# lukecavabarrett/pna

Measured on NVIDIA H100. Metric: aggregated edges/sec (PNA layer fwd), higher is better.
Workload: dtype f32

## Files before the change

### include/pna_b200.h

```cpp
#ifndef PNA_B200_H
#define PNA_B200_H

#include <stddef.h>
#include <stdint.h>

#ifdef __cplusplus
extern "C" {
#endif

#define PNA_ABI_VERSION 8

typedef void* pna_stream_t;

enum pna_status {
  PNA_OK = 0,
  PNA_ERR_BAD_ARG = -1,
  PNA_ERR_UNSUPPORTED = -2,
  PNA_ERR_CUDA = -3,
  PNA_ERR_INDEX = -4,
  PNA_ERR_WORKSPACE = -5,
  PNA_ERR_CAPTURING = -6
};

enum pna_dtype { PNA_F32 = 0, PNA_BF16 = 1 };

enum pna_aggr { PNA_AGGR_SUM = 0, PNA_AGGR_MEAN = 1, PNA_AGGR_MIN = 2, PNA_AGGR_MAX = 3, PNA_AGGR_VAR = 4, PNA_AGGR_STD = 5,
                PNA_AGGR_MOMENT3 = 6, PNA_AGGR_MOMENT4 = 7, PNA_AGGR_MOMENT5 = 8,
                PNA_AGGR_SOFTMAX = 9, PNA_AGGR_SOFTMIN = 10, PNA_AGGR_NORMALISED_MEAN = 11,
                PNA_AGGR_SKIP = 15  };
enum pna_scaler { PNA_SCALE_IDENTITY = 0, PNA_SCALE_AMPLIFICATION = 1, PNA_SCALE_ATTENUATION = 2, PNA_SCALE_LINEAR = 3, PNA_SCALE_INVERSE_LINEAR = 4 };

#define PNA_MAX_AGGR 6
#define PNA_MAX_SCALERS 5

enum pna_flags {
  PNA_FLAG_ZERO_ISOLATED = 1u,
  PNA_FLAG_SKIP_LIGHT = 2u,
  PNA_FLAG_SKIP_HUBS = 4u,
  PNA_FLAG_GATHER_L1 = 16u,
  PNA_FLAG_RELU_VAR = 8u
};

enum pna_query_what {
  PNA_QUERY_ABI_VERSION = 0,
  PNA_QUERY_SM_ARCH = 1,
  PNA_QUERY_DEFAULT_SPLIT = 2,
  PNA_QUERY_DEFAULT_CHUNK = 3,
  PNA_QUERY_DEVICE_SM_COUNT = 4,
  PNA_QUERY_MAX_FEATURES = 5,
  PNA_QUERY_SIZEOF_CSR = 6,
  PNA_QUERY_SIZEOF_AGG = 7
};

typedef struct pna_csr {
  int64_t n_nodes;
  int64_t n_edges;
  int32_t split_threshold;
  int32_t chunk_edges;
  int32_t* rowptr;
  int32_t* col;
  int32_t* perm;
  int32_t* hub_info;
  int32_t* chunk_items;
  int64_t cap_hubs;
  int64_t cap_chunks;
  int64_t n_hubs;
  int64_t n_chunks;
  int32_t max_degree;
  int32_t n_part;
  int32_t* light_rowptr;
  int32_t* light_deg;
  int32_t* light_col;
// ... 154 lines not shown
```

### pna_b200/_lib.py

```python
from __future__ import annotations

import ctypes as C
import os
import subprocess
import threading

_HERE = os.path.dirname(os.path.abspath(__file__))
REPO_ROOT = os.path.dirname(_HERE)
LIB_PATH = os.environ.get("PNA_B200_LIB") or os.path.join(_HERE, "libpna_sm90.so")
CUDA_SOURCES = [os.path.join(_HERE, "csrc", n) for n in
                ("pna_aggregate.cu", "pna_aggregate_f32_vec.cu", "pna_aggregate_f32_scalar.cu", "pna_aggregate_bf16_vec.cu",
                 "pna_aggregate_bf16_scalar.cu", "pna_aggregate_bwd.cu", "pna_linear.cu", "pna_csr.cu", "pna_peer.cu", "pna_misc.cu",
                 "pna_edge_mlp.cu")]
CUDA_HEADERS = [os.path.join(_HERE, "csrc", n) for n in ("common.cuh", "pna_aggregate.cuh", "pna_aggregate_impl.cuh",
                                                                   "pna_aggregate_moments.cuh", "pna_aggregate_weighted.cuh")] + [
    os.path.join(REPO_ROOT, "include", "pna_b200.h")]
BUILD_DIR = os.path.join(_HERE, "csrc", "build")

NVCC_FLAGS = ["-gencode", "arch=compute_90a,code=sm_90a", "-lineinfo", "-O3", "-std=c++17", "-fmad=false", "-Xcompiler", "-fPIC"]

ABI_VERSION = 8
PNA_OK = 0
PNA_ERR_CAPTURING = -6
PNA_F32, PNA_BF16 = 0, 1
AGGR_CODES = {"sum": 0, "mean": 1, "min": 2, "max": 3, "var": 4, "std": 5, "_skip": 15}
MOMENTS = ("moment3", "moment4", "moment5")
WEIGHTED = ("softmax", "softmin", "normalised_mean")
ALL_AGGR_CODES = {**AGGR_CODES, "moment3": 6, "moment4": 7, "moment5": 8, "softmax": 9, "softmin": 10, "normalised_mean": 11}
SCALER_CODES = {"identity": 0, "amplification": 1, "attenuation": 2, "linear": 3, "inverse_linear": 4}
FLAG_ZERO_ISOLATED, FLAG_SKIP_LIGHT, FLAG_SKIP_HUBS, FLAG_RELU_VAR, FLAG_GATHER_L1 = 1, 2, 4, 8, 16
(QUERY_ABI_VERSION, QUERY_SM_ARCH, QUERY_DEFAULT_SPLIT, QUERY_DEFAULT_CHUNK, QUERY_DEVICE_SM_COUNT,
 QUERY_MAX_FEATURES, QUERY_SIZEOF_CSR, QUERY_SIZEOF_AGG) = range(8)
EDGE_MLP_MAX_WIDTH = 64

EXPORTED_SYMBOLS = ("pna_csr_workspace_bytes", "pna_csr_build", "pna_csr_light_view", "pna_csr_light_view_workspace_bytes", "pna_aggregate_fwd", "pna_aggregate_bwd",
                    "pna_aggregate_bwd_coef", "pna_aggregate_bwd_combine", "pna_aggregate_bwd_slots", "pna_aggregate_bwd_peer_slots",
                    "pna_gather_rows", "pna_halo_pull", "pna_halo_grad_pull", "pna_peer_barrier", "pna_linear_fwd", "pna_linear_scaled_fwd", "pna_row_scales", "pna_linear_workspace_bytes",
                    "pna_linear_bwd_workspace_bytes", "pna_linear_bwd_data", "pna_linear_bwd_weight", "pna_edge_mlp_fwd",
                    "pna_edge_mlp_bwd", "pna_edge_msg_fwd", "pna_edge_msg_bwd", "pna_query", "pna_last_error",
                    "pna_linear_towers_scaled_fwd", "pna_linear_towers_bwd_data", "pna_edge_msg_fwd_bf16", "pna_edge_msg_bwd_bf16",
                    "pna_linear_towers_scaled_fwd_bf16")


class PnaError(RuntimeError):

    def __init__(self, status: int, message: str):
        super().__init__(f"libpna_sm90 status {status}: {message}")
        self.status = status


class CsrStruct(C.Structure):
    _fields_ = [
        ("n_nodes", C.c_int64), ("n_edges", C.c_int64),
        ("split_threshold", C.c_int32), ("chunk_edges", C.c_int32),
        ("rowptr", C.c_void_p), ("col", C.c_void_p), ("perm", C.c_void_p),
        ("hub_info", C.c_void_p), ("chunk_items", C.c_void_p),
        ("cap_hubs", C.c_int64), ("cap_chunks", C.c_int64),
        ("n_hubs", C.c_int64), ("n_chunks", C.c_int64),
        ("max_degree", C.c_int32), ("n_part", C.c_int32),
        ("light_rowptr", C.c_void_p), ("light_deg", C.c_void_p), ("light_col", C.c_void_p), ("part", C.c_void_p),
        ("n_light_edges", C.c_int64), ("n_src_nodes", C.c_int64), ("hot_source_fraction", C.c_float), ("reserved", C.c_int32),
    ]

# ... 190 lines not shown
```

### pna_b200/aggregate.py

```python
from __future__ import annotations

import ctypes as C
import os
from typing import Mapping, Optional, Sequence, Union

import torch

from . import _lib, capture
from .csr import CSRGraph

_DTYPES = {torch.float32: _lib.PNA_F32, torch.bfloat16: _lib.PNA_BF16}
Names = Union[str, Sequence[str]]


def _names(v: Names) -> list:
    return v.split() if isinstance(v, str) else list(v)


def _ptr(t: Optional[torch.Tensor]):
    return None if t is None else t.data_ptr()


def _rows2d(t: torch.Tensor, what: str) -> torch.Tensor:
    if t.dim() != 2:
        raise ValueError(f"{what} must be 2-D, got shape {tuple(t.shape)}")
    if t.size(1) > 1 and t.stride(1) != 1:
        t = t.contiguous()
    if t.size(0) > 1 and t.stride(0) < t.size(1):
        t = t.contiguous()
    return t


HOT_SOURCE_FRACTION_FOR_L1 = 0.25


DYNAMIC_TAIL_MIN_PARTITION_COST = 256


def _dynamic_tail(csr: CSRGraph) -> bool:
    return csr.n_part > 0 and (csr.n_edges + 12 * csr.n_nodes) / csr.n_part >= DYNAMIC_TAIL_MIN_PARTITION_COST


def _check_scaler_degree(t: torch.Tensor, n_rows: int, dev) -> torch.Tensor:
    if t.dtype != torch.int32 or t.device != dev or t.numel() != n_rows or not t.is_contiguous():
        raise ValueError("scaler_degree must be a contiguous int32 [n_rows] tensor on the same device")
    return t


def _check_degree_col(t: torch.Tensor, n_edges: int, dev) -> torch.Tensor:
    if t.dtype != torch.int32 or t.device != dev or t.numel() != n_edges or not t.is_contiguous():
        raise ValueError("degree_col must be a contiguous int32 [n_edges] tensor on the same device")
    return t


def fold_finalize_enabled() -> bool:
    return os.environ.get("PNA_B200_FOLD_FINALIZE", "0") == "1"


def boundary_dtype() -> Optional[torch.dtype]:
    if not torch.is_autocast_enabled("cuda"):
        return None
    return torch.bfloat16 if torch.get_autocast_dtype("cuda") == torch.bfloat16 else torch.float32


def at_boundary(t: Optional[torch.Tensor]) -> Optional[torch.Tensor]:
    if t is not None and t.dtype == torch.float16 and boundary_dtype() is not None:
        return t.float()
    return t

# ... 27 lines not shown
    N = csr.n_nodes
    if F % towers != 0:
        raise ValueError(f"feature width {F} not divisible by towers={towers}")
    Ft = F // towers
    if messages_in_csr_order:
        if gathered.size(0) != csr.n_edges:
            raise ValueError("messages_in_csr_order needs one row per CSR slot")
    n_aggr, aggr_codes = _lib.pack_codes(aggregators, _lib.ALL_AGGR_CODES, "aggregator")
    n_scal, scal_codes = _lib.pack_codes(scalers, _lib.SCALER_CODES, "scaler")
    if row_bias is not None:
        row_bias = _rows2d(row_bias.to(gathered.dtype), "row_bias")
        if tuple(row_bias.shape) != (N, F):
            raise ValueError(f"row_bias must be [{N}, {F}]")
    if self_feat is not None:
        self_feat = _rows2d(self_feat.to(gathered.dtype), "self_feat")
        need = F if self_divided else Ft
        if self_feat.size(0) != N or self_feat.size(1) != need:
            raise ValueError(f"self_feat must be [{N}, {need}]")
    width = towers * output_width(Ft, n_aggr, n_scal, self_feat is not None)
    if out is None:
        out = torch.empty((N, width), dtype=gathered.dtype, device=dev)
    else:
        if out.dtype != gathered.dtype or out.device != dev or out.dim() != 2 or out.size(0) != N or out.size(1) < width \
                or out.stride(1) != 1:
            raise ValueError("bad `out` buffer")
    if row_ids is not None:
        if row_ids.dtype != torch.int32 or not row_ids.is_contiguous() or row_ids.device != dev:
            raise ValueError("row_ids must be a contiguous int32 tensor on the same device")
    if gather_l1 is None:
        gather_l1 = (not messages_in_csr_order) and peer is None and csr.hot_source_fraction > HOT_SOURCE_FRACTION_FOR_L1
    flags = (_lib.FLAG_GATHER_L1 if gather_l1 else 0) | \
            (_lib.FLAG_ZERO_ISOLATED if zero_isolated else 0) | (_lib.FLAG_SKIP_LIGHT if skip_light else 0) | \
            (_lib.FLAG_SKIP_HUBS if skip_hubs else 0) | (_lib.FLAG_RELU_VAR if relu_var else 0)
    partials = None if skip_hubs else csr.hub_partials(F)
    d = _lib.AggStruct(
        gathered=_ptr(gathered), ld_gathered=gathered.stride(0) if gathered.size(0) > 1 else F,
        rowptr=_ptr(csr.rowptr), col=None if messages_in_csr_order else (_ptr(csr.col) if csr.n_edges else None),
        row_bias=_ptr(row_bias), ld_row_bias=0 if row_bias is None else (row_bias.stride(0) if N > 1 else F),
        self_feat=_ptr(self_feat), ld_self=0 if self_feat is None else (self_feat.stride(0) if N > 1 else self_feat.size(1)),
        self_tower_stride=Ft if (self_feat is not None and self_divided) else 0,
        out=_ptr(out), ld_out=out.stride(0) if N > 1 else out.size(1),
        n_rows=N, n_feat=F, n_towers=towers, dtype=_DTYPES[gathered.dtype],
        n_aggr=n_aggr, aggr_codes=aggr_codes, n_scalers=n_scal, scaler_codes=scal_codes,
        avg_log=float(avg_deg["log"]), avg_lin=float(avg_deg.get("lin", 1.0)),
        flags=flags, split_threshold=csr.split_threshold, chunk_edges=csr.chunk_edges,
        hub_info=_ptr(csr.hub_info) if csr.n_hubs else None, chunk_items=_ptr(csr.chunk_items) if csr.n_hubs else None,
        n_hubs=csr.n_hubs, n_chunks=csr.n_chunks, hub_partials=_ptr(partials), max_degree=int(csr.max_degree),
        row_ids=_ptr(row_ids), n_row_ids=0 if row_ids is None else int(row_ids.numel()))
    if scaler_degree is not None:
        d.scaler_degree = _check_scaler_degree(scaler_degree, N, dev).data_ptr()
    if degree_col is not None:
        d.degree_col = _check_degree_col(degree_col, csr.n_edges, dev).data_ptr()
    if view is None and row_ids is None and _dynamic_tail(csr):
        d.work_counter = _ptr(csr.work_counter())
    if view is None and row_ids is None:
        view = csr.full_view()
        if fold_finalize_enabled() and not skip_hubs and peer is None:
            d.hub_done = _ptr(csr.hub_done())
    if view is not None and row_ids is None and N > 0:
        d.light_rowptr, d.light_deg, d.part, d.n_part = _ptr(view.light_rowptr), _ptr(view.light_deg), _ptr(view.part), view.n_part
        d.light_col = _ptr(view.light_col) if csr.n_edges else None
        d.n_view_rows = view.n_view_rows or N
    if peer is not None:
        ptr_table, shift = peer
        if ptr_table.dtype != torch.int64 or ptr_table.device != dev:
            raise ValueError("peer pointer table must be an int64 tensor on the same device")
# ... 194 lines not shown
```

### pna_b200/csrc/common.cuh

```cuda
#pragma once
#include <cuda_runtime.h>
#include <cuda_bf16.h>
#include <stdint.h>
#include <stdio.h>
#include <stdarg.h>
#include "../../include/pna_b200.h"

#if defined(__CUDA_ARCH__) && (__CUDA_ARCH__ != 900)
#error "libpna_sm90 is written for sm_90a (H100) only"
#endif

namespace pna {

void set_error(const char* fmt, ...);
int cuda_fail(cudaError_t e, const char* what);

#define PNA_CUDA_TRY(expr)                                   \
  do {                                                       \
    cudaError_t _e = (expr);                                 \
    if (_e != cudaSuccess) return ::pna::cuda_fail(_e, #expr); \
  } while (0)

#define PNA_REQUIRE(cond, code, ...)      \
  do {                                    \
// ... 32 lines not shown
    }
  }
};
__device__ __forceinline__ DegScales deg_scales(int deg, float avg_log, float avg_lin) {
  const bool iso = deg == 0;
  const float degf = (float)deg;
  const float lg = logf(degf + 1.0f);
  DegScales s;
  s.amp = __fdiv_rn(lg, avg_log);
  s.att = iso ? 1.0f : __fdiv_rn(avg_log, lg);
  s.lin = __fdiv_rn(degf, avg_lin);
  s.ilin = iso ? 1.0f : __fdiv_rn(avg_lin, degf);
  return s;
}

template <typename V>
__device__ __forceinline__ void store_out(V* p, V v) { __stcs(p, v); }

template <typename T, int VEC>
struct Io;

template <>
struct Io<float, 4> {
  typedef float4 Raw;
  static __device__ __forceinline__ Raw load_raw(const float* p) { return __ldg(reinterpret_cast<const float4*>(p)); }
  static __device__ __forceinline__ void unpack(const Raw& r, float (&v)[4]) { v[0] = r.x; v[1] = r.y; v[2] = r.z; v[3] = r.w; }
  static __device__ __forceinline__ void load(const float* p, float (&v)[4]) { unpack(load_raw(p), v); }
  static __device__ __forceinline__ void store(float* p, const float (&v)[4]) {
    store_out(reinterpret_cast<float4*>(p), make_float4(v[0], v[1], v[2], v[3]));
  }
};

template <>
struct Io<float, 1> {
  typedef float Raw;
  static __device__ __forceinline__ Raw load_raw(const float* p) { return __ldg(p); }
  static __device__ __forceinline__ void unpack(const Raw& r, float (&v)[1]) { v[0] = r; }
  static __device__ __forceinline__ void load(const float* p, float (&v)[1]) { v[0] = __ldg(p); }
  static __device__ __forceinline__ void store(float* p, const float (&v)[1]) { __stcs(p, v[0]); }
};

template <>
struct Io<__nv_bfloat16, 8> {
  typedef uint4 Raw;
  static __device__ __forceinline__ Raw load_raw(const __nv_bfloat16* p) { return __ldg(reinterpret_cast<const uint4*>(p)); }
  static __device__ __forceinline__ void load(const __nv_bfloat16* p, float (&v)[8]) { unpack(load_raw(p), v); }
  static __device__ __forceinline__ void unpack(const Raw& r, float (&v)[8]) {
    v[0] = __uint_as_float(r.x << 16); v[1] = __uint_as_float(r.x & 0xffff0000u);
    v[2] = __uint_as_float(r.y << 16); v[3] = __uint_as_float(r.y & 0xffff0000u);
    v[4] = __uint_as_float(r.z << 16); v[5] = __uint_as_float(r.z & 0xffff0000u);
    v[6] = __uint_as_float(r.w << 16); v[7] = __uint_as_float(r.w & 0xffff0000u);
  }
  static __device__ __forceinline__ unsigned pack(float lo, float hi) {
    const __nv_bfloat162 b = __floats2bfloat162_rn(lo, hi);
    return *reinterpret_cast<const unsigned*>(&b);
  }
  static __device__ __forceinline__ void store(__nv_bfloat16* p, const float (&v)[8]) {
    uint4 r;
    r.x = pack(v[0], v[1]); r.y = pack(v[2], v[3]); r.z = pack(v[4], v[5]); r.w = pack(v[6], v[7]);
    store_out(reinterpret_cast<uint4*>(p), r);
  }
};

template <>
struct Io<__nv_bfloat16, 1> {
  typedef unsigned short Raw;
// ... 11 lines not shown
```

### pna_b200/csrc/pna_aggregate_impl.cuh

```cuda
#pragma once
#include "pna_aggregate.cuh"

namespace pna {

constexpr int kThreads = 256;
constexpr int min_blocks(int vec, int k) { return vec * k <= 4 ? 4 : (vec * k <= 8 ? 3 : (vec * k <= 16 ? 2 : 1)); }

template <int VEC>
__device__ __forceinline__ void store_f32(float* p, const float (&v)[VEC]) {
  if constexpr (VEC % 4 == 0) {
#pragma unroll
    for (int i = 0; i < VEC; i += 4) *reinterpret_cast<float4*>(p + i) = make_float4(v[i], v[i + 1], v[i + 2], v[i + 3]);
  } else {
#pragma unroll
    for (int i = 0; i < VEC; ++i) p[i] = v[i];
  }
}

template <typename T, int VEC, int G, int K, int U, typename Cfg>
__global__ void __launch_bounds__(kThreads, min_blocks(VEC, K)) k_rows(const KParams p) {
  constexpr int RPW = 32 / G;
  const int lane = threadIdx.x & 31;
  const int gl = lane % G;
  const long long slot = ((long long)blockIdx.x * (kThreads / 32) + (threadIdx.x >> 5)) * RPW + lane / G;
  long long row;
  if (p.row_ids) {
    if (slot >= p.n_row_ids) return;
    row = __ldg(p.row_ids + slot);
  } else {
    if (slot >= p.n_rows) return;
    row = slot;
  }
  const int beg = __ldg(p.rowptr + row), end = __ldg(p.rowptr + row + 1);
// ... 158 lines not shown
              }
            }
        }
      }
    }

#pragma unroll
    for (int u = 0; u < U; ++u) {
      const int src = __shfl_sync(FULL, cvN, gbase + u);
      if (u < dN) {
#pragma unroll
        for (int k = 0; k < K; ++k)
          if (fm.ok[k]) raw[u][k] = Io<T, VEC>::load_raw((PEER ? gathered_row<T>(p, src) : local_row<T>(p, src)) + fm.f[k]);
      }
    }
    if (deg >= 0) finalize_row_ds<T, VEC, G, K, Cfg>(p, fm, (long long)row, deg, scales_of_row(s_scale_lut, p, row, deg), acc);

    row = rowN; beg = begN; deg = degN; d = dN; cv = cvN;
    if (has_bias) {
#pragma unroll
      for (int k = 0; k < K; ++k)
#pragma unroll
        for (int i = 0; i < VEC; ++i) bias[BIAS ? k : 0][i] = biasN[BIAS ? k : 0][i];
    }
  }
}

constexpr int kStreamThreads = 128;

__device__ __forceinline__ unsigned smem_u32(const void* ptr) { return (unsigned)__cvta_generic_to_shared(ptr); }

template <typename T, int VEC>
__device__ __forceinline__ typename Io<T, VEC>::Raw lds_raw(unsigned addr) {
  static_assert(sizeof(typename Io<T, VEC>::Raw) == 16, "the stream path moves 128-bit chunks");
  typename Io<T, VEC>::Raw r;
  unsigned* w = reinterpret_cast<unsigned*>(&r);
  unsigned a, b, c, d;
  asm volatile("ld.shared.v4.b32 {%0, %1, %2, %3}, [%4];" : "=r"(a), "=r"(b), "=r"(c), "=r"(d) : "r"(addr));
  w[0] = a; w[1] = b; w[2] = c; w[3] = d;
  return r;
}

template <typename T, int VEC, int K, int DEPTH = 1>
struct StreamGeom {
  static constexpr int kHalfBytes = 4096;
  static constexpr int kStages = 2;
  static constexpr int kBlockBytes = 32 * VEC * K * (int)sizeof(T);
  static constexpr int kHalf = kHalfBytes * DEPTH;
  static constexpr int kH = (kHalf / kBlockBytes) < 4 ? 4 : ((kHalf / kBlockBytes) > 32 ? 32 : (kHalf / kBlockBytes));
  static constexpr int kWarpBytes = kStages * kH * kBlockBytes;
  static constexpr size_t kSmem = (size_t)(kStreamThreads / 32) * kWarpBytes;
};

template <bool L1 = false>
__device__ __forceinline__ void cp_async16(unsigned dst, const void* src, unsigned long long policy) {
  if constexpr (L1)
    asm volatile("cp.async.ca.shared.global.L2::cache_hint [%0], [%1], 16, %2;" ::"r"(dst), "l"(__cvta_generic_to_global(src)), "l"(policy)
                 : "memory");
  else
    asm volatile("cp.async.cg.shared.global.L2::cache_hint [%0], [%1], 16, %2;" ::"r"(dst), "l"(__cvta_generic_to_global(src)), "l"(policy)
                 : "memory");
}
__device__ __forceinline__ void cp_async_commit() { asm volatile("cp.async.commit_group;" ::: "memory"); }
template <int N>
__device__ __forceinline__ void cp_async_wait() { asm volatile("cp.async.wait_group %0;" ::"n"(N) : "memory"); }
__device__ __forceinline__ unsigned long long l2_policy_evict_last() {
  unsigned long long pol;
  asm volatile("createpolicy.fractional.L2::evict_last.b64 %0, 1.0;" : "=l"(pol));
  return pol;
}

constexpr int kFinGroups = 8;

template <int VEC, int K, int UF>
__device__ __forceinline__ void merge_partials(const float* __restrict__ base, long long F, const int (&f)[K], const bool (&ok)[K],
                                               int first, int count, int stride, Acc<VEC> (&acc)[K]) {
  for (int j = 0; j < count; j += UF) {
    float ps[UF][K][4][VEC];
#pragma unroll
    for (int u = 0; u < UF; ++u) {
// ... 57 lines not shown
    if (lane == 0) t = atomicAdd(ctr, 1);
    return __shfl_sync(FULL, t, 0);
  };
  if (nch > kFinGroups) {
    const int g = jc % kFinGroups;
    const int mine = (nch - g + kFinGroups - 1) / kFinGroups;
    if (arrive(cnt + g) != mine - 1) return;
    if (lane == 0) cnt[g] = 0;
    __threadfence();
#pragma unroll
    for (int k = 0; k < K; ++k) acc[k].init();
    merge_partials<VEC, K, UFm>(p.partials, p.F, fm.f, fm.ok, first + g, mine, kFinGroups, acc);
    float* __restrict__ part = p.partials + (long long)(first + g) * 4ll * p.F;
#pragma unroll
    for (int k = 0; k < K; ++k) {
      if (!fm.ok[k]) continue;
      store_f32<VEC>(part + 0ll * p.F + fm.f[k], acc[k].sum);
      store_f32<VEC>(part + 1ll * p.F + fm.f[k], acc[k].sq);
      store_f32<VEC>(part + 2ll * p.F + fm.f[k], acc[k].mn);
      store_f32<VEC>(part + 3ll * p.F + fm.f[k], acc[k].mx);
    }
    if (arrive(cnt + 8) != kFinGroups - 1) return;
  } else if (arrive(cnt + 8) != nch - 1) {
    return;
  }
  if (lane == 0) cnt[8] = 0;
  __threadfence();
#pragma unroll
  for (int k = 0; k < K; ++k) acc[k].init();
  merge_partials<VEC, K, UFm>(p.partials, p.F, fm.f, fm.ok, first, nch > kFinGroups ? kFinGroups : nch, 1, acc);
  finalize_row<T, VEC, G, K, Cfg>(p, fm, (long long)__ldg(p.hub_info + 4 * h), __ldg(p.hub_info + 4 * h + 3), acc);
}

template <typename T, int VEC, int K, typename Cfg, bool BIAS, int DEPTH, bool FOLD = false, bool L1 = false>
__global__ void __launch_bounds__(kStreamThreads, tiled_min_blocks(VEC, K)) k_rows_stream(const __grid_constant__ KParams p) {
  constexpr int G = 32;
  constexpr int H = StreamGeom<T, VEC, K, DEPTH>::kH;
  constexpr int SLOT = StreamGeom<T, VEC, K, DEPTH>::kBlockBytes;
  constexpr int NST = StreamGeom<T, VEC, K, DEPTH>::kStages;
  constexpr int CB = 16;
  constexpr unsigned FULL = 0xffffffffu;
  constexpr bool PEER = DEPTH > 1;
  extern __shared__ __align__(128) unsigned char smem[];
  __shared__ float4 s_scale_lut[kScaleLut];
  const int lane = threadIdx.x & 31;
  const int warp = threadIdx.x >> 5;
  fill_scale_lut(s_scale_lut, p, threadIdx.x, kStreamThreads);

  const unsigned ring = smem_u32(smem) + warp * StreamGeom<T, VEC, K, DEPTH>::kWarpBytes;
  const unsigned long long keep = l2_policy_evict_last();

  const long long W = (long long)gridDim.x * (kStreamThreads / 32);
  const long long w = (long long)blockIdx.x * (kStreamThreads / 32) + warp;
  const int n_static = p.work_ctr ? p.n_static : p.n_part;
  int pi_a = (int)((w * n_static) / W), pi_b = (int)(((w + 1) * n_static) / W);
#pragma unroll 1
 for (;;) {
  const int pa = __ldg(p.part + pi_a);
  const int pb = __ldg(p.part + pi_b);
  const int Q0 = __ldg(p.lrowptr + pa);
  const int Te = __ldg(p.lrowptr + pb) - Q0;
  if (pa < pb) {
  const int* __restrict__ lcol = p.lcol + Q0;
  const int fblock = blockIdx.y * (G * VEC * K);
  FeatMap<VEC, G, K> fm;
  fm.init(p, lane, fblock);

  auto source_of = [&](int q) -> int { return (lane < H && q < Te) ? __ldg(lcol + q) : 0; };
  const int lane_elems = fblock + lane * VEC;
  const char* const xlane = reinterpret_cast<const char*>(static_cast<const T*>(p.x) + lane_elems);
  const unsigned ldxb = (unsigned)p.ldx * (unsigned)sizeof(T);
  auto issue_half = [&](int stage, int src) {
    unsigned dst = ring + (unsigned)(stage * H) * SLOT + lane * CB;
#pragma unroll
    for (int u = 0; u < H; ++u, dst += SLOT) {
      const int s_u = __shfl_sync(FULL, src, u);
      const char* sp;
      if constexpr (PEER) sp = reinterpret_cast<const char*>(gathered_row<T>(p, s_u) + lane_elems);
      else sp = xlane + (unsigned long long)(unsigned)s_u * ldxb;
#pragma unroll
      for (int k = 0; k < K; ++k)
        if (fm.ok[k]) cp_async16<L1>(dst + k * (32 * CB), sp + k * (32 * CB), keep);
    }
    cp_async_commit();
  };

  int pend = source_of(lane);
  if (Te > 0) {
#pragma unroll
    for (int s0 = 0; s0 < NST; ++s0) {
      issue_half(s0, pend);
      pend = source_of((s0 + 1) * H + lane);
    }
  }
  int stage = 0;
  int n_issued = NST;

  auto load_deg = [&](int r) -> int { return (r + lane < pb) ? __ldg(p.ldeg + r + lane) : -1; };
  const ViewMap vmap = {p.n_rows, (int)(p.n_view_rows - p.n_rows)};
  auto load_rid = [&](int r) -> int {
    if (p.row_ids) return (r + lane < pb) ? __ldg(p.row_ids + r + lane) : 0;
    return (int)vmap.to_row(r + lane);
  };
  int dg = load_deg(pa), rid = load_rid(pa);

  const unsigned lane_off = (unsigned)lane * (unsigned)CB;
  int q = 0;
#pragma unroll 1
  for (int r0 = pa; r0 < pb; r0 += 32) {
    const int dgN = load_deg(r0 + 32), ridN = load_rid(r0 + 32);
    const int nj = min(32, pb - r0);
#pragma unroll 1
    for (int j = 0; j < nj; ++j) {
      const int deg = __shfl_sync(FULL, dg, j);
      if (deg < 0) continue;
      const int row = __shfl_sync(FULL, rid, j);
      const bool chunk_row = row >= p.n_rows;
      float bias[BIAS ? K : 1][VEC];
      if (BIAS) {
        long long brow = row;
        if (chunk_row) brow = __ldg(p.hub_info + 4 * __ldg(p.chunk_items + 2 * (row - (int)p.n_rows)));
#pragma unroll
        for (int k = 0; k < K; ++k)
          if (fm.ok[k]) Io<T, VEC>::load(static_cast<const T*>(p.bias) + brow * p.ldb + fm.f[k], bias[BIAS ? k : 0]);
      }
      Acc<VEC> acc[K];
#pragma unroll
      for (int k = 0; k < K; ++k) acc[k].init();

      int left = deg;
      while (left > 0) {
        const int inhalf = q & (H - 1);
        if (inhalf == 0) {
          cp_async_wait<NST - 1>();
        }
        const int seg = min(left, H - inhalf);
        unsigned sp = ring + (unsigned)(stage * H + inhalf) * SLOT + lane_off;
        int t = 0;
        for (; t + 2 <= seg; t += 2, sp += 2 * SLOT) {
#pragma unroll
          for (int k = 0; k < K; ++k) {
            if (fm.ok[k]) {
              float m0[VEC], m1[VEC];
              Io<T, VEC>::unpack(lds_raw<T, VEC>(sp + k * (32 * CB)), m0);
              Io<T, VEC>::unpack(lds_raw<T, VEC>(sp + SLOT + k * (32 * CB)), m1);
              acc[k].template add2<BIAS>(m0, m1, bias[BIAS ? k : 0]);
            }
          }
        }
        if (t < seg) {
#pragma unroll
          for (int k = 0; k < K; ++k) {
            if (fm.ok[k]) {
              float m0[VEC];
              Io<T, VEC>::unpack(lds_raw<T, VEC>(sp + k * (32 * CB)), m0);
              acc[k].template add1<BIAS>(m0, bias[BIAS ? k : 0]);
            }
          }
        }
        q += seg;
        left -= seg;
        if ((q & (H - 1)) == 0 || q == Te) {
          issue_half(stage, pend);
          pend = source_of((n_issued + 1) * H + lane);
          ++n_issued;
          stage = (stage + 1 == NST) ? 0 : stage + 1;
        }
      }
      if (!chunk_row) {
        if (Cfg::kStatic && deg == 0 && !p.sdeg) {
          finalize_isolated_row<T, VEC, G, K, Cfg>(p, fm, (long long)row, scales_of_row(s_scale_lut, p, row, 0));
        } else {
          finalize_row_ds<T, VEC, G, K, Cfg>(p, fm, (long long)row, deg, scales_of_row(s_scale_lut, p, row, deg), acc);
        }
      } else {
        float* __restrict__ part = p.partials + (long long)(row - (int)p.n_rows) * 4ll * p.F;
#pragma unroll
        for (int k = 0; k < K; ++k) {
          if (!fm.ok[k]) continue;
          store_f32<VEC>(part + 0ll * p.F + fm.f[k], acc[k].sum);
          store_f32<VEC>(part + 1ll * p.F + fm.f[k], acc[k].sq);
          store_f32<VEC>(part + 2ll * p.F + fm.f[k], acc[k].mn);
          store_f32<VEC>(part + 3ll * p.F + fm.f[k], acc[k].mx);
        }
        if constexpr (FOLD) fold_split_row<T, VEC, K, Cfg>(p, row - (int)p.n_rows, fblock);
      }
    }
    dg = dgN; rid = ridN;
  }
  if (p.work_ctr) { cp_async_wait<0>(); __syncwarp(); }
  }
  if (!p.work_ctr) break;
  int g = 0;
  if (lane == 0) g = atomicAdd(p.work_ctr, 1);
  g = __shfl_sync(FULL, g, 0);
  pi_a = n_static + g;
  if (pi_a >= p.n_part) break;
  pi_b = pi_a + 1;
 }
}

template <typename T, int VEC, int G, int K, int U>
__global__ void __launch_bounds__(kThreads, min_blocks(VEC, K)) k_hub_chunks(const KParams p) {
  constexpr int RPW = 32 / G;
  const int lane = threadIdx.x & 31;
  const int gl = lane % G;
  const long long c = ((long long)blockIdx.x * (kThreads / 32) + (threadIdx.x >> 5)) * RPW + lane / G;
  if (c >= p.n_chunks) return;
  const int h = __ldg(p.chunk_items + 2 * c), j = __ldg(p.chunk_items + 2 * c + 1);
  const long long row = __ldg(p.hub_info + 4 * h);
  const int rbeg = __ldg(p.rowptr + row), rend = __ldg(p.rowptr + row + 1);
  const int beg = rbeg + j * p.chunk;
  const int end = min(beg + p.chunk, rend);

  FeatMap<VEC, G, K> fm;
  fm.init(p, gl, blockIdx.y * (G * VEC * K));
  Acc<VEC> acc[K];
  float bias[K][VEC];
#pragma unroll
  for (int k = 0; k < K; ++k) {
    acc[k].init();
    if (p.bias && fm.ok[k]) Io<T, VEC>::load(static_cast<const T*>(p.bias) + row * p.ldb + fm.f[k], bias[k]);
  }
// ... 141 lines not shown
    if (q != 0) return;
#pragma unroll
    for (int k = 0; k < K; ++k) acc[k].init();
    merge_partials<VEC, K, UF>(p.partials, p.F, fm.f, fm.ok, first, kFinGroups, 1, acc);
  } else {
    if (q != 0) return;
    merge_partials<VEC, K, UF>(p.partials, p.F, fm.f, fm.ok, first, nch, 1, acc);
  }
  finalize_row<T, VEC, G, K, CfgDynamic>(p, fm, row, deg, acc);
}

template <typename T, int VEC, int G, int K, int U>
static int launch_config(const KParams& p_in, cudaStream_t st) {
  constexpr int RPW = 32 / G;
  constexpr int per_block = (kThreads / 32) * RPW;
  KParams p = p_in;
  const unsigned gy = (unsigned)((p.F + G * VEC * K - 1) / (G * VEC * K));
  if (gy != 1 || !(p.n_view_rows > p.n_rows) || p.hub_merged) p.hub_done = nullptr;
  bool folded = false;
  bool chunks_in_stream = false;
  if (!(p.flags & PNA_FLAG_SKIP_LIGHT)) {
    const long long slots = p.row_ids ? p.n_row_ids : p.n_rows;
    if (slots > 0) {
      const long long gx = (slots + per_block - 1) / per_block;
      PNA_REQUIRE(gx <= 0x7fffffffll, PNA_ERR_UNSUPPORTED, "too many rows for one launch: %lld", slots);
      const unsigned std_s = (0u) | (1u << 4) | (2u << 8);
      const bool s3 = p.nS == 3 && (p.scodes & 0xfffu) == std_s && p.nA == 4;
      const bool s1 = p.nS == 1 && (p.scodes & 0xfu) == PNA_SCALE_IDENTITY && p.nA == 4;
      const int cfg = (p.acodes & 0xffffu) != CfgMeanMaxMinStd::ACODES ? 0 : s3 ? 1 : s1 ? 2 : 0;
      if (G == 32 && VEC > 1 && p.lrowptr != nullptr && p.col != nullptr) {
       if constexpr (G == 32 && VEC > 1) {
        const bool b = p.bias != nullptr;
        const bool deep = p.peer_x != nullptr;
#define PNA_LAUNCH_STREAM_(CFG, B, DEPTH, FOLD) PNA_LAUNCH_STREAM__(CFG, B, DEPTH, FOLD, false)
#define PNA_LAUNCH_STREAM__(CFG, B, DEPTH, FOLD, L1)                                                                    \
  do {                                                                                                             \
    constexpr size_t smem = StreamGeom<T, VEC, K, DEPTH>::kSmem;                                                   \
    auto kern = k_rows_stream<T, VEC, K, CFG, B, DEPTH, FOLD, L1>;                                                     \
    static int resident = 0;                  \
    if (resident == 0) {         \
      PNA_CUDA_TRY(cudaFuncSetAttribute(kern, cudaFuncAttributeMaxDynamicSharedMemorySize, (int)smem));            \
      int dev = 0, sms = 0, nb = 0;                                                                                \
      PNA_CUDA_TRY(cudaGetDevice(&dev));                                                                           \
      PNA_CUDA_TRY(cudaDeviceGetAttribute(&sms, cudaDevAttrMultiProcessorCount, dev));                             \
      PNA_CUDA_TRY(cudaOccupancyMaxActiveBlocksPerMultiprocessor(&nb, kern, kStreamThreads, smem));                \
      resident = (nb > 0 ? nb : 1) * sms;                                                                          \
    }                                                                                                              \
    long long gxs = (slots + 8 * (kStreamThreads / 32) - 1) / (8 * (kStreamThreads / 32));  \
    if (gxs > resident) gxs = resident;                                                                            \
    if (gxs < 1) gxs = 1;                                                                                          \
    if (p.work_ctr) {     \
      const long long nw = gxs * (kStreamThreads / 32);                                                            \
      p.n_static = (int)((long long)p.n_part * 7 / 10);                                                            \
      if (gy != 1 || p.n_static < nw || gxs < resident) p.work_ctr = nullptr;                                      \
      else PNA_CUDA_TRY(cudaMemsetAsync(p.work_ctr, 0, sizeof(int), st));                                          \
    }                                                                                                              \
    kern<<<dim3((unsigned)gxs, gy), kStreamThreads, smem, st>>>(p);                                                \
  } while (0)
#define PNA_LAUNCH_STREAM(CFG, B)                                        \
  do {                                                                   \
    if (p.hub_done) PNA_LAUNCH_STREAM_(CFG, B, 1, true);                 \
    else PNA_LAUNCH_STREAM_(CFG, B, 1, false);                           \
  } while (0)
        if (deep) {
          p.hub_done = nullptr;
          if (cfg == 1 && !b) PNA_LAUNCH_STREAM_(CfgMeanMaxMinStd, false, 2, false);
          else if (!b) PNA_LAUNCH_STREAM_(CfgDynamic, false, 2, false);
          else PNA_LAUNCH_STREAM_(CfgDynamic, true, 2, false);
        } else if ((p.flags & PNA_FLAG_GATHER_L1) && cfg == 1 && !b) {
          p.hub_done = nullptr;
          PNA_LAUNCH_STREAM__(CfgMeanMaxMinStd, false, 1, false, true);
        } else if ((p.flags & PNA_FLAG_GATHER_L1) && cfg == 2 && !b) {
          p.hub_done = nullptr;
          PNA_LAUNCH_STREAM__(CfgMeanMaxMinStdId, false, 1, false, true);
        } else if (cfg == 1 && !b) PNA_LAUNCH_STREAM(CfgMeanMaxMinStd, false);
        else if (cfg == 1) PNA_LAUNCH_STREAM(CfgMeanMaxMinStd, true);
        else if (cfg == 2 && !b) PNA_LAUNCH_STREAM(CfgMeanMaxMinStdId, false);
        else if (!b) PNA_LAUNCH_STREAM(CfgDynamic, false);
        else PNA_LAUNCH_STREAM(CfgDynamic, true);
        chunks_in_stream = p.n_view_rows > p.n_rows;
        folded = chunks_in_stream && p.hub_done != nullptr;
#undef PNA_LAUNCH_STREAM
#undef PNA_LAUNCH_STREAM_
#undef PNA_LAUNCH_STREAM__
       }
      } else if constexpr (G >= U && G % U == 0) {
        constexpr int TR = (8 * RPW < 32) ? 8 * RPW : 32;
        constexpr int tiles_per_block = kTiledThreads / 32;
        const long long tiles = (slots + TR - 1) / TR;
        const long long gt = (tiles + tiles_per_block - 1) / tiles_per_block;
        PNA_REQUIRE(gt <= 0x7fffffffll, PNA_ERR_UNSUPPORTED, "too many rows for one launch: %lld", slots);
        const dim3 grid((unsigned)gt, gy);
        const bool b = p.bias != nullptr;
        if (p.peer_x != nullptr) {
          if (!b) k_rows_tiled<T, VEC, G, K, U, CfgDynamic, false, true><<<grid, kTiledThreads, 0, st>>>(p);
          else k_rows_tiled<T, VEC, G, K, U, CfgDynamic, true, true><<<grid, kTiledThreads, 0, st>>>(p);
        } else if (cfg == 1 && !b) k_rows_tiled<T, VEC, G, K, U, CfgMeanMaxMinStd, false><<<grid, kTiledThreads, 0, st>>>(p);
        else if (cfg == 1) k_rows_tiled<T, VEC, G, K, U, CfgMeanMaxMinStd, true><<<grid, kTiledThreads, 0, st>>>(p);
        else if (!b) k_rows_tiled<T, VEC, G, K, U, CfgDynamic, false><<<grid, kTiledThreads, 0, st>>>(p);
        else k_rows_tiled<T, VEC, G, K, U, CfgDynamic, true><<<grid, kTiledThreads, 0, st>>>(p);
      } else {
        k_rows<T, VEC, G, K, U, CfgDynamic><<<dim3((unsigned)gx, gy), kThreads, 0, st>>>(p);
      }
      PNA_CUDA_TRY(cudaGetLastError());
    }
  }
  if (!(p.flags & PNA_FLAG_SKIP_HUBS) && p.n_hubs > 0) {
    if (!chunks_in_stream) {
      const long long gc = (p.n_chunks + per_block - 1) / per_block;
      k_hub_chunks<T, VEC, G, K, U><<<dim3((unsigned)gc, gy), kThreads, 0, st>>>(p);
      PNA_CUDA_TRY(cudaGetLastError());
    }
    if (!folded) {
      if constexpr (G == 32) {
        if (p.hub_merged) {
          for (long long S = 1; S < p.n_chunks; S *= kTreeR) {
            const long long blocks = (p.n_chunks + kTreeR * S - 1) / (kTreeR * S);
// ... 30 lines not shown
```

Before: 2.019 billion.

## Add slab-pass streaming aggregation so gathered feature slices stay L2-resident

Adds a SLAB mode to the stream aggregation kernel. Each warp loops over 256-byte feature slabs of every row, one full pass over its edges per slab, so the source features touched in a pass fit in L2 when the whole gathered matrix does not. It is enabled by default for fp32 inputs without bias when the gathered tensor exceeds 48 MiB but one slab per source fits. In exchange the edge lists and row metadata are re-read once per slab, each row is finalized with narrower float2 vectors, and the launch drops the feature-block grid dimension and the hub folding path.

```diff
diff --git a/include/pna_b200.h b/include/pna_b200.h
--- a/include/pna_b200.h
+++ b/include/pna_b200.h
@@ -38,6 +38,7 @@
   PNA_FLAG_SKIP_LIGHT = 2u,
   PNA_FLAG_SKIP_HUBS = 4u,
   PNA_FLAG_GATHER_L1 = 16u,
+  PNA_FLAG_SLAB_PASSES = 32u,
   PNA_FLAG_RELU_VAR = 8u
 };
 
diff --git a/pna_b200/_lib.py b/pna_b200/_lib.py
--- a/pna_b200/_lib.py
+++ b/pna_b200/_lib.py
@@ -28,7 +28,7 @@
 WEIGHTED = ("softmax", "softmin", "normalised_mean")
 ALL_AGGR_CODES = {**AGGR_CODES, "moment3": 6, "moment4": 7, "moment5": 8, "softmax": 9, "softmin": 10, "normalised_mean": 11}
 SCALER_CODES = {"identity": 0, "amplification": 1, "attenuation": 2, "linear": 3, "inverse_linear": 4}
-FLAG_ZERO_ISOLATED, FLAG_SKIP_LIGHT, FLAG_SKIP_HUBS, FLAG_RELU_VAR, FLAG_GATHER_L1 = 1, 2, 4, 8, 16
+FLAG_ZERO_ISOLATED, FLAG_SKIP_LIGHT, FLAG_SKIP_HUBS, FLAG_RELU_VAR, FLAG_GATHER_L1, FLAG_SLAB_PASSES = 1, 2, 4, 8, 16, 32
 (QUERY_ABI_VERSION, QUERY_SM_ARCH, QUERY_DEFAULT_SPLIT, QUERY_DEFAULT_CHUNK, QUERY_DEVICE_SM_COUNT,
  QUERY_MAX_FEATURES, QUERY_SIZEOF_CSR, QUERY_SIZEOF_AGG) = range(8)
 EDGE_MLP_MAX_WIDTH = 64
diff --git a/pna_b200/aggregate.py b/pna_b200/aggregate.py
--- a/pna_b200/aggregate.py
+++ b/pna_b200/aggregate.py
@@ -35,6 +35,21 @@
 
 
 DYNAMIC_TAIL_MIN_PARTITION_COST = 256
+
+
+SLAB_PASSES_BY_DEFAULT = True
+L2_GATHER_BYTES = 48 << 20
+SLAB_BYTES = 256
+
+
+def slab_passes(gathered: torch.Tensor) -> bool:
+    force = os.environ.get("PNA_B200_SLAB")
+    if force in ("0", "1"):
+        return force == "1"
+    if not SLAB_PASSES_BY_DEFAULT or gathered.dtype != torch.float32:
+        return False
+    n_src, F = gathered.size(0), gathered.size(1)
+    return n_src * F * 4 > L2_GATHER_BYTES and n_src * SLAB_BYTES <= L2_GATHER_BYTES
 
 
 def _dynamic_tail(csr: CSRGraph) -> bool:
@@ -128,6 +143,8 @@
     flags = (_lib.FLAG_GATHER_L1 if gather_l1 else 0) | \
             (_lib.FLAG_ZERO_ISOLATED if zero_isolated else 0) | (_lib.FLAG_SKIP_LIGHT if skip_light else 0) | \
             (_lib.FLAG_SKIP_HUBS if skip_hubs else 0) | (_lib.FLAG_RELU_VAR if relu_var else 0)
+    if not messages_in_csr_order and slab_passes(gathered):
+        flags |= _lib.FLAG_SLAB_PASSES
     partials = None if skip_hubs else csr.hub_partials(F)
     d = _lib.AggStruct(
         gathered=_ptr(gathered), ld_gathered=gathered.stride(0) if gathered.size(0) > 1 else F,
diff --git a/pna_b200/csrc/common.cuh b/pna_b200/csrc/common.cuh
--- a/pna_b200/csrc/common.cuh
+++ b/pna_b200/csrc/common.cuh
@@ -88,6 +88,17 @@
 };
 
 template <>
+struct Io<float, 2> {
+  typedef float2 Raw;
+  static __device__ __forceinline__ Raw load_raw(const float* p) { return __ldg(reinterpret_cast<const float2*>(p)); }
+  static __device__ __forceinline__ void unpack(const Raw& r, float (&v)[2]) { v[0] = r.x; v[1] = r.y; }
+  static __device__ __forceinline__ void load(const float* p, float (&v)[2]) { unpack(load_raw(p), v); }
+  static __device__ __forceinline__ void store(float* p, const float (&v)[2]) {
+    store_out(reinterpret_cast<float2*>(p), make_float2(v[0], v[1]));
+  }
+};
+
+template <>
 struct Io<float, 1> {
   typedef float Raw;
   static __device__ __forceinline__ Raw load_raw(const float* p) { return __ldg(p); }
diff --git a/pna_b200/csrc/pna_aggregate_impl.cuh b/pna_b200/csrc/pna_aggregate_impl.cuh
--- a/pna_b200/csrc/pna_aggregate_impl.cuh
+++ b/pna_b200/csrc/pna_aggregate_impl.cuh
@@ -1,4 +1,5 @@
 #pragma once
+#include <type_traits>
 #include "pna_aggregate.cuh"
 
 namespace pna {
@@ -223,20 +224,28 @@
 
 template <typename T, int VEC>
 __device__ __forceinline__ typename Io<T, VEC>::Raw lds_raw(unsigned addr) {
-  static_assert(sizeof(typename Io<T, VEC>::Raw) == 16, "the stream path moves 128-bit chunks");
   typename Io<T, VEC>::Raw r;
   unsigned* w = reinterpret_cast<unsigned*>(&r);
-  unsigned a, b, c, d;
-  asm volatile("ld.shared.v4.b32 {%0, %1, %2, %3}, [%4];" : "=r"(a), "=r"(b), "=r"(c), "=r"(d) : "r"(addr));
-  w[0] = a; w[1] = b; w[2] = c; w[3] = d;
+  if constexpr (sizeof(r) == 4) {
+    asm volatile("ld.shared.b32 %0, [%1];" : "=r"(w[0]) : "r"(addr));
+  } else if constexpr (sizeof(r) == 8) {
+    asm volatile("ld.shared.v2.b32 {%0, %1}, [%2];" : "=r"(w[0]), "=r"(w[1]) : "r"(addr));
+  } else {
+    static_assert(sizeof(r) == 16, "the stream path moves 128-bit chunks");
+    unsigned a, b, c, d;
+    asm volatile("ld.shared.v4.b32 {%0, %1, %2, %3}, [%4];" : "=r"(a), "=r"(b), "=r"(c), "=r"(d) : "r"(addr));
+    w[0] = a; w[1] = b; w[2] = c; w[3] = d;
+  }
   return r;
 }
 
-template <typename T, int VEC, int K, int DEPTH = 1>
+constexpr int kSlabBytes = 256;
+
+template <typename T, int VEC, int K, int DEPTH = 1, bool SLAB = false>
 struct StreamGeom {
   static constexpr int kHalfBytes = 4096;
   static constexpr int kStages = 2;
-  static constexpr int kBlockBytes = 32 * VEC * K * (int)sizeof(T);
+  static constexpr int kBlockBytes = SLAB ? kSlabBytes : 32 * VEC * K * (int)sizeof(T);
   static constexpr int kHalf = kHalfBytes * DEPTH;
   static constexpr int kH = (kHalf / kBlockBytes) < 4 ? 4 : ((kHalf / kBlockBytes) > 32 ? 32 : (kHalf / kBlockBytes));
   static constexpr int kWarpBytes = kStages * kH * kBlockBytes;
@@ -360,13 +369,17 @@
   finalize_row<T, VEC, G, K, Cfg>(p, fm, (long long)__ldg(p.hub_info + 4 * h), __ldg(p.hub_info + 4 * h + 3), acc);
 }
 
-template <typename T, int VEC, int K, typename Cfg, bool BIAS, int DEPTH, bool FOLD = false, bool L1 = false>
+template <typename T, int VEC, int K, typename Cfg, bool BIAS, int DEPTH, bool FOLD = false, bool L1 = false, bool SLAB = false>
 __global__ void __launch_bounds__(kStreamThreads, tiled_min_blocks(VEC, K)) k_rows_stream(const __grid_constant__ KParams p) {
   constexpr int G = 32;
-  constexpr int H = StreamGeom<T, VEC, K, DEPTH>::kH;
-  constexpr int SLOT = StreamGeom<T, VEC, K, DEPTH>::kBlockBytes;
-  constexpr int NST = StreamGeom<T, VEC, K, DEPTH>::kStages;
+  using Geom = StreamGeom<T, VEC, K, DEPTH, SLAB>;
+  constexpr int H = Geom::kH;
+  constexpr int SLOT = Geom::kBlockBytes;
+  constexpr int NST = Geom::kStages;
   constexpr int CB = 16;
+  constexpr int RV = SLAB ? kSlabBytes / (32 * (int)sizeof(T)) : VEC;
+  constexpr int RK = SLAB ? 1 : K;
+  static_assert(!SLAB || (sizeof(T) == 4 && !BIAS && DEPTH == 1 && !FOLD && !L1), "slab passes: fp32, no bias, local rows");
   constexpr unsigned FULL = 0xffffffffu;
   constexpr bool PEER = DEPTH > 1;
   extern __shared__ __align__(128) unsigned char smem[];
@@ -375,7 +388,7 @@
   const int warp = threadIdx.x >> 5;
   fill_scale_lut(s_scale_lut, p, threadIdx.x, kStreamThreads);
 
-  const unsigned ring = smem_u32(smem) + warp * StreamGeom<T, VEC, K, DEPTH>::kWarpBytes;
+  const unsigned ring = smem_u32(smem) + warp * Geom::kWarpBytes;
   const unsigned long long keep = l2_policy_evict_last();
 
   const long long W = (long long)gridDim.x * (kStreamThreads / 32);
@@ -390,8 +403,10 @@
   const int Te = __ldg(p.lrowptr + pb) - Q0;
   if (pa < pb) {
   const int* __restrict__ lcol = p.lcol + Q0;
-  const int fblock = blockIdx.y * (G * VEC * K);
-  FeatMap<VEC, G, K> fm;
+#pragma unroll 1
+  for (int fs = 0; fs < (SLAB ? p.F : 1); fs += kSlabBytes / (int)sizeof(T)) {
+  const int fblock = SLAB ? fs : blockIdx.y * (G * VEC * K);
+  FeatMap<RV, G, RK> fm;
   fm.init(p, lane, fblock);
 
   auto source_of = [&](int q) -> int { return (lane < H && q < Te) ? __ldg(lcol + q) : 0; };
@@ -399,6 +414,20 @@
   const char* const xlane = reinterpret_cast<const char*>(static_cast<const T*>(p.x) + lane_elems);
   const unsigned ldxb = (unsigned)p.ldx * (unsigned)sizeof(T);
   auto issue_half = [&](int stage, int src) {
+    if constexpr (SLAB) {
+      constexpr int CPS = kSlabBytes / CB;
+      const int c = lane % CPS, ul = lane / CPS;
+      const bool inside = fblock + c * (CB / (int)sizeof(T)) < p.F;
+      const char* const xs = reinterpret_cast<const char*>(static_cast<const T*>(p.x) + fblock) + c * CB;
+      unsigned dst = ring + (unsigned)(stage * H + ul) * SLOT + c * CB;
+#pragma unroll
+      for (int u = 0; u < H; u += 32 / CPS, dst += (32 / CPS) * SLOT) {
+        const int s_u = __shfl_sync(FULL, src, u + ul);
+        if (inside) cp_async16<false>(dst, xs + (unsigned long long)(unsigned)s_u * ldxb, keep);
+      }
+      cp_async_commit();
+      return;
+    }
     unsigned dst = ring + (unsigned)(stage * H) * SLOT + lane * CB;
 #pragma unroll
     for (int u = 0; u < H; ++u, dst += SLOT) {
@@ -432,7 +461,7 @@
   };
   int dg = load_deg(pa), rid = load_rid(pa);
 
-  const unsigned lane_off = (unsigned)lane * (unsigned)CB;
+  const unsigned lane_off = (unsigned)lane * (unsigned)(RV * sizeof(T));
   int q = 0;
 #pragma unroll 1
   for (int r0 = pa; r0 < pb; r0 += 32) {
@@ -444,44 +473,45 @@
       if (deg < 0) continue;
       const int row = __shfl_sync(FULL, rid, j);
       const bool chunk_row = row >= p.n_rows;
-      float bias[BIAS ? K : 1][VEC];
+      float bias[BIAS ? RK : 1][RV];
       if (BIAS) {
         long long brow = row;
         if (chunk_row) brow = __ldg(p.hub_info + 4 * __ldg(p.chunk_items + 2 * (row - (int)p.n_rows)));
 #pragma unroll
-        for (int k = 0; k < K; ++k)
-          if (fm.ok[k]) Io<T, VEC>::load(static_cast<const T*>(p.bias) + brow * p.ldb + fm.f[k], bias[BIAS ? k : 0]);
-      }
-      Acc<VEC> acc[K];
-#pragma unroll
-      for (int k = 0; k < K; ++k) acc[k].init();
+        for (int k = 0; k < RK; ++k)
+          if (fm.ok[k]) Io<T, RV>::load(static_cast<const T*>(p.bias) + brow * p.ldb + fm.f[k], bias[BIAS ? k : 0]);
+      }
+      Acc<RV> acc[RK];
+#pragma unroll
+      for (int k = 0; k < RK; ++k) acc[k].init();
 
       int left = deg;
       while (left > 0) {
         const int inhalf = q & (H - 1);
         if (inhalf == 0) {
           cp_async_wait<NST - 1>();
+          if constexpr (SLAB) __syncwarp();
         }
         const int seg = min(left, H - inhalf);
         unsigned sp = ring + (unsigned)(stage * H + inhalf) * SLOT + lane_off;
         int t = 0;
         for (; t + 2 <= seg; t += 2, sp += 2 * SLOT) {
 #pragma unroll
-          for (int k = 0; k < K; ++k) {
+          for (int k = 0; k < RK; ++k) {
             if (fm.ok[k]) {
-              float m0[VEC], m1[VEC];
-              Io<T, VEC>::unpack(lds_raw<T, VEC>(sp + k * (32 * CB)), m0);
-              Io<T, VEC>::unpack(lds_raw<T, VEC>(sp + SLOT + k * (32 * CB)), m1);
+              float m0[RV], m1[RV];
+              Io<T, RV>::unpack(lds_raw<T, RV>(sp + k * (32 * CB)), m0);
+              Io<T, RV>::unpack(lds_raw<T, RV>(sp + SLOT + k * (32 * CB)), m1);
               acc[k].template add2<BIAS>(m0, m1, bias[BIAS ? k : 0]);
             }
           }
         }
         if (t < seg) {
 #pragma unroll
-          for (int k = 0; k < K; ++k) {
+          for (int k = 0; k < RK; ++k) {
             if (fm.ok[k]) {
-              float m0[VEC];
-              Io<T, VEC>::unpack(lds_raw<T, VEC>(sp + k * (32 * CB)), m0);
+              float m0[RV];
+              Io<T, RV>::unpack(lds_raw<T, RV>(sp + k * (32 * CB)), m0);
               acc[k].template add1<BIAS>(m0, bias[BIAS ? k : 0]);
             }
           }
@@ -489,6 +519,7 @@
         q += seg;
         left -= seg;
         if ((q & (H - 1)) == 0 || q == Te) {
+          if constexpr (SLAB) __syncwarp();
           issue_half(stage, pend);
           pend = source_of((n_issued + 1) * H + lane);
           ++n_issued;
@@ -497,26 +528,27 @@
       }
       if (!chunk_row) {
         if (Cfg::kStatic && deg == 0 && !p.sdeg) {
-          finalize_isolated_row<T, VEC, G, K, Cfg>(p, fm, (long long)row, scales_of_row(s_scale_lut, p, row, 0));
+          finalize_isolated_row<T, RV, G, RK, Cfg>(p, fm, (long long)row, scales_of_row(s_scale_lut, p, row, 0));
         } else {
-          finalize_row_ds<T, VEC, G, K, Cfg>(p, fm, (long long)row, deg, scales_of_row(s_scale_lut, p, row, deg), acc);
+          finalize_row_ds<T, RV, G, RK, Cfg>(p, fm, (long long)row, deg, scales_of_row(s_scale_lut, p, row, deg), acc);
         }
       } else {
         float* __restrict__ part = p.partials + (long long)(row - (int)p.n_rows) * 4ll * p.F;
 #pragma unroll
-        for (int k = 0; k < K; ++k) {
+        for (int k = 0; k < RK; ++k) {
           if (!fm.ok[k]) continue;
-          store_f32<VEC>(part + 0ll * p.F + fm.f[k], acc[k].sum);
-          store_f32<VEC>(part + 1ll * p.F + fm.f[k], acc[k].sq);
-          store_f32<VEC>(part + 2ll * p.F + fm.f[k], acc[k].mn);
-          store_f32<VEC>(part + 3ll * p.F + fm.f[k], acc[k].mx);
+          store_f32<RV>(part + 0ll * p.F + fm.f[k], acc[k].sum);
+          store_f32<RV>(part + 1ll * p.F + fm.f[k], acc[k].sq);
+          store_f32<RV>(part + 2ll * p.F + fm.f[k], acc[k].mn);
+          store_f32<RV>(part + 3ll * p.F + fm.f[k], acc[k].mx);
         }
         if constexpr (FOLD) fold_split_row<T, VEC, K, Cfg>(p, row - (int)p.n_rows, fblock);
       }
     }
     dg = dgN; rid = ridN;
   }
-  if (p.work_ctr) { cp_async_wait<0>(); __syncwarp(); }
+  if (SLAB || p.work_ctr) { cp_async_wait<0>(); __syncwarp(); }
+  }
   }
   if (!p.work_ctr) break;
   int g = 0;
@@ -724,11 +756,14 @@
        if constexpr (G == 32 && VEC > 1) {
         const bool b = p.bias != nullptr;
         const bool deep = p.peer_x != nullptr;
+        constexpr bool kSlabKernels = std::is_same<T, float>::value && VEC == 4;
+        const bool use_slab = kSlabKernels && (p.flags & PNA_FLAG_SLAB_PASSES) && !b;
 #define PNA_LAUNCH_STREAM_(CFG, B, DEPTH, FOLD) PNA_LAUNCH_STREAM__(CFG, B, DEPTH, FOLD, false)
-#define PNA_LAUNCH_STREAM__(CFG, B, DEPTH, FOLD, L1)                                                                    \
+#define PNA_LAUNCH_STREAM__(CFG, B, DEPTH, FOLD, L1) PNA_LAUNCH_STREAM___(CFG, B, DEPTH, FOLD, L1, false, K)
+#define PNA_LAUNCH_STREAM___(CFG, B, DEPTH, FOLD, L1, SLAB, KK)                                                       \
   do {                                                                                                             \
-    constexpr size_t smem = StreamGeom<T, VEC, K, DEPTH>::kSmem;                                                   \
-    auto kern = k_rows_stream<T, VEC, K, CFG, B, DEPTH, FOLD, L1>;                                                     \
+    constexpr size_t smem = StreamGeom<T, VEC, KK, DEPTH, SLAB>::kSmem;                                            \
+    auto kern = k_rows_stream<T, VEC, KK, CFG, B, DEPTH, FOLD, L1, SLAB>;                                          \
     static int resident = 0;                  \
     if (resident == 0) {         \
       PNA_CUDA_TRY(cudaFuncSetAttribute(kern, cudaFuncAttributeMaxDynamicSharedMemorySize, (int)smem));            \
@@ -741,13 +776,14 @@
     long long gxs = (slots + 8 * (kStreamThreads / 32) - 1) / (8 * (kStreamThreads / 32));  \
     if (gxs > resident) gxs = resident;                                                                            \
     if (gxs < 1) gxs = 1;                                                                                          \
+    const unsigned gyk = SLAB ? 1u : gy;                         \
     if (p.work_ctr) {     \
       const long long nw = gxs * (kStreamThreads / 32);                                                            \
       p.n_static = (int)((long long)p.n_part * 7 / 10);                                                            \
-      if (gy != 1 || p.n_static < nw || gxs < resident) p.work_ctr = nullptr;                                      \
+      if (gyk != 1 || p.n_static < nw || gxs < resident) p.work_ctr = nullptr;                                     \
       else PNA_CUDA_TRY(cudaMemsetAsync(p.work_ctr, 0, sizeof(int), st));                                          \
     }                                                                                                              \
-    kern<<<dim3((unsigned)gxs, gy), kStreamThreads, smem, st>>>(p);                                                \
+    kern<<<dim3((unsigned)gxs, gyk), kStreamThreads, smem, st>>>(p);                                               \
   } while (0)
 #define PNA_LAUNCH_STREAM(CFG, B)                                        \
   do {                                                                   \
@@ -765,6 +801,12 @@
         } else if ((p.flags & PNA_FLAG_GATHER_L1) && cfg == 2 && !b) {
           p.hub_done = nullptr;
           PNA_LAUNCH_STREAM__(CfgMeanMaxMinStdId, false, 1, false, true);
+        } else if (use_slab && cfg == 1) {
+          p.hub_done = nullptr;
+          if constexpr (kSlabKernels) PNA_LAUNCH_STREAM___(CfgMeanMaxMinStd, false, 1, false, false, true, 1);
+        } else if (use_slab && cfg == 2) {
+          p.hub_done = nullptr;
+          if constexpr (kSlabKernels) PNA_LAUNCH_STREAM___(CfgMeanMaxMinStdId, false, 1, false, false, true, 1);
         } else if (cfg == 1 && !b) PNA_LAUNCH_STREAM(CfgMeanMaxMinStd, false);
         else if (cfg == 1) PNA_LAUNCH_STREAM(CfgMeanMaxMinStd, true);
         else if (cfg == 2 && !b) PNA_LAUNCH_STREAM(CfgMeanMaxMinStdId, false);
@@ -775,6 +817,7 @@
 #undef PNA_LAUNCH_STREAM
 #undef PNA_LAUNCH_STREAM_
 #undef PNA_LAUNCH_STREAM__
+#undef PNA_LAUNCH_STREAM___
        }
       } else if constexpr (G >= U && G % U == 0) {
         constexpr int TR = (8 * RPW < 32) ? 8 * RPW : 32;
```

Result: faster. 2.048 billion (median of 6 runs) (+1.5%).
